# jan-van-bergen/GPU-Raytracer

Hardware: AMD Instinct MI355X
Metric: Mrays/s (primary+secondary) + ms/frame, Sponza 1920x1080 4spp BVH8 (higher is better)
Workload: dtype f32

## Files before the change

gpu-raytracer_amd/__init__.py:

```python
import ctypes
import fcntl
import os
import tarfile
import tempfile
from ctypes import POINTER, byref, c_char_p, c_double, c_float, c_int, c_int32, c_size_t, c_uint8, c_uint32, c_void_p

import numpy as np

_HERE = os.path.dirname(os.path.abspath(__file__))
REPO_ROOT = os.path.dirname(_HERE)
ASSET_DIR = os.path.join(REPO_ROOT, "assets")
DEVICE_LIB_PATH = os.environ.get("GRT_DEVICE_LIB") or os.path.join(_HERE, "csrc", "libgrt_device.so")
HOST_LIB_PATH = os.path.join(_HERE, "host", "libgrt_host.so")

RT_MAX_BOUNCES = 128
RT_BATCH_SIZE = 1080 * 720
AOV_RADIANCE, AOV_RADIANCE_DIRECT, AOV_RADIANCE_INDIRECT, AOV_ALBEDO, AOV_NORMAL, AOV_POSITION, AOV_COUNT = range(7)
MATERIAL_LIGHT, MATERIAL_DIFFUSE, MATERIAL_PLASTIC, MATERIAL_DIELECTRIC, MATERIAL_CONDUCTOR = range(5)
FILTER_BOX, FILTER_TENT, FILTER_GAUSSIAN = range(3)


class GPUConfig(ctypes.Structure):
    _fields_ = [("reconstruction_filter", c_int32), ("aov_mask", c_uint32), ("num_bounces", c_int32),
                ("enable_mipmapping", c_int32), ("enable_next_event_estimation", c_int32),
# ... 23 lines not shown

_device = None
_host = None


def device_lib():
    global _device
    if _device is None:
        if not os.path.exists(DEVICE_LIB_PATH):
            raise DeviceLibraryMissing("%s is missing -- run `python __graft_entry__.py` (build()) first" % DEVICE_LIB_PATH)
        lib = ctypes.CDLL(DEVICE_LIB_PATH, mode=ctypes.RTLD_GLOBAL)
        if hasattr(lib, "rt_abi_version") and lib.rt_abi_version() != 17:
            raise DeviceLibraryMissing("%s has ABI version %d, this front end was written for 17 -- rebuild (python __graft_entry__.py)" % (DEVICE_LIB_PATH, lib.rt_abi_version()))
        lib.rt_last_error.restype = c_char_p
        lib.rt_last_error.argtypes = [c_void_p]
        lib.rt_version.restype = c_char_p
        lib.rt_create.argtypes = [c_int, POINTER(c_void_p)]
        lib.rt_destroy.argtypes = [c_void_p]
        fp, u32p, u8p = POINTER(c_float), POINTER(c_uint32), POINTER(c_uint8)
        lib.rt_trace_rays.argtypes = [c_void_p] + [c_void_p] * 6 + [c_size_t, c_void_p, c_int, POINTER(c_float)]
        lib.rt_trace_shadow_rays.argtypes = [c_void_p] + [c_void_p] * 7 + [c_size_t, c_void_p, c_int, POINTER(c_float)]
        lib.rt_trace_stream_rays.argtypes = [c_void_p, c_int] + [c_void_p] * 6 + [c_size_t, c_void_p] + [c_void_p] * 7 + [c_size_t, c_void_p, c_void_p, c_void_p]
        lib.rt_generate_rays.argtypes = [c_void_p, c_int, c_int, c_int] + [c_void_p] * 7
        lib.rt_random_samples.argtypes = [c_void_p, c_int, c_void_p, c_size_t, c_uint32, c_uint32, c_void_p]
        lib.rt_sample_texture.argtypes = [c_void_p, c_int, c_int, c_void_p, c_size_t, c_void_p]
        lib.rt_sample_table.argtypes = [c_void_p, c_void_p, c_int, c_int, c_int, c_int, c_void_p, c_size_t, c_void_p]
        lib.rt_sample_sky.argtypes = [c_void_p, c_void_p, c_size_t, c_void_p]
        lib.rt_sample_sky_distribution.argtypes = [c_void_p, c_void_p, c_size_t, c_void_p]
        lib.rt_sky_pdf.argtypes = [c_void_p, c_void_p, c_size_t, c_void_p]
        lib.rt_bsdf_eval.argtypes = [c_void_p, c_int, c_void_p, c_size_t, c_void_p]
        lib.rt_bsdf_sample.argtypes = [c_void_p, c_int, c_void_p, c_size_t, c_void_p]
        lib.rt_sample_lights.argtypes = [c_void_p, c_void_p, c_size_t, c_int, c_void_p]
        lib.rt_sort_rays.argtypes = [c_void_p, c_int, c_int, c_int, c_void_p, c_size_t, c_void_p, c_size_t, c_void_p, c_size_t, c_size_t, c_uint32] + [c_void_p] * 9
        lib.rt_upload_lights.argtypes = [c_void_p, c_void_p, c_void_p, c_size_t, c_void_p, c_void_p, c_void_p, c_size_t, c_float]
        lib.rt_upload_material_normal_maps.argtypes = [c_void_p, c_void_p, c_size_t]
        lib.rt_set_bvh_type.argtypes = [c_void_p, c_int]
        lib.rt_upload_material_opacity.argtypes = [c_void_p, c_void_p, c_void_p, c_void_p, c_size_t]
        lib.rt_read_material_opacity.argtypes = [c_void_p, c_int, c_void_p, c_size_t, POINTER(c_int), POINTER(c_int)]
        lib.rt_perturb_normals.argtypes = [c_void_p, c_int, c_void_p, c_size_t, c_void_p]
        lib.rt_set_sky_sampling.argtypes = [c_void_p, c_float]
        lib.rt_set_sky.argtypes = [c_void_p, c_void_p, c_int, c_int, c_float]
        lib.rt_upload_media.argtypes = [c_void_p, c_void_p, c_size_t]
        lib.rt_upload_instances.argtypes = [c_void_p] + [c_void_p] * 5 + [c_size_t]
        lib.rt_upload_materials.argtypes = [c_void_p, c_void_p, c_void_p, c_size_t]
        lib.rt_set_pixel_query.argtypes = [c_void_p, c_int]
        lib.rt_set_svgf_matrices.argtypes = [c_void_p, c_void_p, c_void_p]
# ... 714 lines not shown
    _dev_check(ctx, device_lib().rt_trace_shadow_rays(ctx, o[0].ctypes.data, o[1].ctypes.data, o[2].ctypes.data, d[0].ctypes.data, d[1].ctypes.data, d[2].ctypes.data, m.ctypes.data, n, occluded.ctypes.data, repeat, byref(ms)))
    return occluded, ms.value


def trace_stream_rays(ctx, iteration, origin, direction, hits, shadow_origin, shadow_direction, max_distance, counting=False):
    o, d = _f32(origin).reshape(3, -1), _f32(direction).reshape(3, -1)
    so, sd, m = _f32(shadow_origin).reshape(3, -1), _f32(shadow_direction).reshape(3, -1), _f32(max_distance).reshape(-1)
    n, k = o.shape[1], so.shape[1]
    if d.shape[1] != n or sd.shape[1] != k or m.size != k:
        raise ValueError("trace_stream_rays: ray arrays of different lengths")
    out = np.array(hits, np.uint32, order="C", copy=True).reshape(n, 4)
    light = np.zeros(k, np.float32)
    stats = np.zeros(10, np.uint64) if counting else None
    info = np.zeros(4, np.int32)
    _dev_check(ctx, device_lib().rt_trace_stream_rays(ctx, iteration, o[0].ctypes.data, o[1].ctypes.data, o[2].ctypes.data, d[0].ctypes.data, d[1].ctypes.data, d[2].ctypes.data, n, out.ctypes.data,
                                                      so[0].ctypes.data, so[1].ctypes.data, so[2].ctypes.data, sd[0].ctypes.data, sd[1].ctypes.data, sd[2].ctypes.data, m.ctypes.data, k, light.ctypes.data,
                                                      stats.ctypes.data if counting else None, info.ctypes.data))
    if counting:
        names = ("nodes", "triangles", "instances_transformed", "instances_identity", "rays")
        stats = {kind: {name: int(stats[5 * j + i]) for i, name in enumerate(names)} for j, kind in enumerate(("closest", "shadow"))}
    return out, light, stats, info


def generate_rays(ctx, sample_index, pixel_offset, pixel_count):
    o = np.zeros((3, pixel_count), np.float32)
    d = np.zeros((3, pixel_count), np.float32)
    px = np.zeros(pixel_count, np.uint32)
    _dev_check(ctx, device_lib().rt_generate_rays(ctx, sample_index, pixel_offset, pixel_count, o[0].ctypes.data, o[1].ctypes.data, o[2].ctypes.data, d[0].ctypes.data, d[1].ctypes.data, d[2].ctypes.data, px.ctypes.data))
    return o, d, px


def random_samples(ctx, dimension, pixel_indices, bounce, sample_index):
    px = np.ascontiguousarray(pixel_indices, dtype=np.uint32)
    out = np.zeros((px.size, 2), np.float32)
    _dev_check(ctx, device_lib().rt_random_samples(ctx, dimension, px.ctypes.data, px.size, bounce, sample_index, out.ctypes.data))
    return out


def sample_texture(ctx, texture_index, filter, args):
    a = _f32(args).reshape(-1, 8)
    out = np.zeros((a.shape[0], 4), np.float32)
    _dev_check(ctx, device_lib().rt_sample_texture(ctx, texture_index, filter, a.ctypes.data, a.shape[0], out.ctypes.data))
    return out


def sample_table(ctx, table, coords):
# ... 282 lines not shown
```

gpu-raytracer_amd/csrc/kernels_shade.hip:

```cpp
#include "rt_shading.h"

#ifndef RT_SHADE_BLOCK
#define RT_SHADE_BLOCK 256
#endif
#ifndef RT_SHADE_WAVES
#define RT_SHADE_WAVES 4
#endif
#ifndef RT_SHADE_ONE_APPEND
#define RT_SHADE_ONE_APPEND 1
#endif
#ifndef RT_OCTANT_BUCKETS
#define RT_OCTANT_BUCKETS 1
#endif
#if RT_OCTANT_BUCKETS
#define RT_RAY_BUCKET(d) direction_octant(d)
#else
#define RT_RAY_BUCKET(d) 0u
#endif
#ifndef RT_SORT_BLOCK
#define RT_SORT_BLOCK 1024
#endif
#ifndef RT_SORT_WAVES
#define RT_SORT_WAVES 8
#endif
// ... 46 lines not shown
	origin = mk3(p.camera.position[0], p.camera.position[1], p.camera.position[2]) + offset;
}

__global__ void __launch_bounds__(RT_SHADE_BLOCK) kernel_generate(RtParams p, int sample_index, int pixel_offset, int pixel_count) {
	const int ray_count = pixel_count * p.batch_samples;
	if (blockIdx.x == 0 && threadIdx.x == 0) p.sizes->trace[0] = ray_count;
	for (int index = blockIdx.x * blockDim.x + threadIdx.x; index < ray_count; index += gridDim.x * blockDim.x) {
		int sample_in_batch = index / pixel_count;
		int index_offset = rt_map_pixel(p, index - sample_in_batch * pixel_count + pixel_offset);
		int x = index_offset % p.screen_width;
		int y = index_offset / p.screen_width;
		int pixel_index = x + y * p.screen_pitch;
		unsigned virtual_pixel = unsigned(sample_in_batch) * p.frame_pixels + unsigned(pixel_index);

		f3 origin, direction;
		camera_generate_ray(p, int(virtual_pixel), sample_index, x, y, origin, direction, sample_index + sample_in_batch);

		store3(p.trace[0].origin,    index, origin);
		store3(p.trace[0].direction, index, direction);
		p.trace[0].pixel_index_and_flags[index] = virtual_pixel;
	}
}

__global__ void __launch_bounds__(RT_SHADE_BLOCK) kernel_generate_stream(RtParams p, int sample_index, int pixel_offset, int pixel_count, int slot_base, int queue_offset, int block_width, int band_rows) {
	const int ray_count = pixel_count * p.batch_samples;
	const RtTraceBuffer & out = p.trace[p.stream_iteration & 1];
	const int base = p.stream->trace_count[p.stream_iteration & 1] + queue_offset;
	for (int index = blockIdx.x * blockDim.x + threadIdx.x; index < ray_count; index += gridDim.x * blockDim.x) {
		int sample_in_batch = index / pixel_count;
		int index_offset = rt_map_pixel(p, index - sample_in_batch * pixel_count + pixel_offset);
		int x = index_offset % p.screen_width;
		int y = index_offset / p.screen_width;
		if (band_rows > 0) {
			int band = y / band_rows;
			int rows = min(band_rows, p.screen_height - band * band_rows);
			int in_band = index_offset - band * band_rows * p.screen_width;
			if (band_rows == 8 && block_width == 8 && rows == 8 && (in_band >> 6) * 8 + 8 <= p.screen_width) {
				x = (in_band >> 6) * 8 + (in_band & 7);
				y = band * 8 + ((in_band >> 3) & 7);
			} else {
				int block = in_band / (block_width * rows);
				int in_block = in_band - block * block_width * rows;
				int columns = min(block_width, p.screen_width - block * block_width);
				x = block * block_width + in_block % columns;
				y = band * band_rows + in_block / columns;
			}
		}
		int pixel_index = x + y * p.screen_pitch;
		unsigned slot = unsigned(slot_base + sample_in_batch);
		unsigned virtual_pixel = slot * p.frame_pixels + unsigned(pixel_index);

		f3 origin, direction;
		camera_generate_ray(p, int(virtual_pixel), sample_index + sample_in_batch - int(slot), x, y, origin, direction, sample_index + sample_in_batch);

		store3(out.origin,    base + index, origin);
		store3(out.direction, base + index, direction);
		out.pixel_index_and_flags[base + index] = virtual_pixel;
	}
}

__global__ void __launch_bounds__(256) kernel_stream_advance(RtStreamControl * control, int iteration, int generated, volatile int * progress, int reset_ring_first, int reset_ring_count) {
	for (int k = int(threadIdx.x); k < reset_ring_count * RT_STAT_KINDS * RT_MAX_BOUNCES; k += int(blockDim.x))
		(&control->stats[(reset_ring_first + k / (RT_STAT_KINDS * RT_MAX_BOUNCES)) % RT_STREAM_SUBMISSIONS][0][0])[k % (RT_STAT_KINDS * RT_MAX_BOUNCES)] = 0;
	const int q = iteration & 1;
	for (int k = int(threadIdx.x); k < 2 * RT_ENDGAME_MAX_WAVES; k += int(blockDim.x)) (&control->endgame[q][0][0])[k] = 0;
	if (threadIdx.x != 0) return;
	int total = control->trace_count[q] + generated;
	control->trace_count[q] = total;
	control->trace_count[q ^ 1] = 0;
	for (int m = 0; m < 4; m++) control->material_count[m] = 0;
	control->shadow_count[q] = 0;
	control->cursor[q][0] = 0; control->cursor[q][1] = 0;
	if (progress) { progress[1] = total; __threadfence_system(); progress[0] = iteration; }
}

__global__ void kernel_expand_bc1(const uint2 * __restrict__ blocks, uchar4 * __restrict__ texels, size_t texel_count) {
// ... 1184 lines not shown
		case 2: hipLaunchKernelGGL(sky ? kernel_material_dielectric_sky_nmap : kernel_material_dielectric_nmap, grid, block, 0, stream, p, bounce, sample_index); break;
		case 3: hipLaunchKernelGGL(sky ? kernel_material_conductor_sky_nmap  : kernel_material_conductor_nmap,  grid, block, 0, stream, p, bounce, sample_index); break;
	}
}
void rt_launch_material(const RtParams & p, int material_slot, int bounce, int sample_index, hipStream_t stream) {
	dim3 grid(2048), block(RT_SHADE_BLOCK);
	if (p.normal_map_slots & (1 << material_slot)) { launch_material_nmap(p, material_slot, bounce, sample_index, stream); return; }
	if (p.sky_nee_share > 0.0f) {
		switch (material_slot) {
			case 0: hipLaunchKernelGGL(p.textures_compressed ? kernel_material_diffuse_sky : kernel_material_diffuse_texels_sky, grid, block, 0, stream, p, bounce, sample_index); break;
			case 1: hipLaunchKernelGGL(p.textures_compressed ? kernel_material_plastic_sky : kernel_material_plastic_texels_sky, grid, block, 0, stream, p, bounce, sample_index); break;
			case 2: hipLaunchKernelGGL(kernel_material_dielectric_sky, grid, block, 0, stream, p, bounce, sample_index); break;
			case 3: hipLaunchKernelGGL(kernel_material_conductor_sky,  grid, block, 0, stream, p, bounce, sample_index); break;
		}
		return;
	}
	switch (material_slot) {
		case 0: if (p.textures_compressed) hipLaunchKernelGGL(kernel_material_diffuse, grid, block, 0, stream, p, bounce, sample_index); else hipLaunchKernelGGL(kernel_material_diffuse_texels, grid, block, 0, stream, p, bounce, sample_index); break;
		case 1: if (p.textures_compressed) hipLaunchKernelGGL(kernel_material_plastic, grid, block, 0, stream, p, bounce, sample_index); else hipLaunchKernelGGL(kernel_material_plastic_texels, grid, block, 0, stream, p, bounce, sample_index); break;
		case 2: hipLaunchKernelGGL(kernel_material_dielectric, grid, block, 0, stream, p, bounce, sample_index); break;
		case 3: hipLaunchKernelGGL(kernel_material_conductor,  grid, block, 0, stream, p, bounce, sample_index); break;
	}
}
void rt_launch_generate_stream(const RtParams & p, int sample_index, int pixel_offset, int pixel_count, int slot_base, int queue_offset, int block_width, int band_rows, hipStream_t stream) {
	hipLaunchKernelGGL(kernel_generate_stream, dim3(streaming_grid(pixel_count * p.batch_samples)), dim3(RT_SHADE_BLOCK), 0, stream, p, sample_index, pixel_offset, pixel_count, slot_base, queue_offset, block_width, band_rows);
}
void rt_launch_stream_advance(RtStreamControl * control, int iteration, int generated, int * progress, int reset_ring_first, int reset_ring_count, hipStream_t stream) {
	hipLaunchKernelGGL(kernel_stream_advance, dim3(1), dim3(256), 0, stream, control, iteration, generated, (volatile int *)progress, reset_ring_first, reset_ring_count);
}
#ifndef RT_STREAM_SHADE_GRID
#define RT_STREAM_SHADE_GRID 8192
#endif
#ifndef RT_STREAM_SORT_GRID
#define RT_STREAM_SORT_GRID 2048
#endif
void rt_launch_sort_stream(const RtParams & p, hipStream_t stream) {
	hipLaunchKernelGGL(p.sky_nee_share > 0.0f ? kernel_sort_stream_sky : kernel_sort_stream, dim3(RT_STREAM_SORT_GRID * RT_SHADE_BLOCK / RT_SORT_BLOCK), dim3(RT_SORT_BLOCK), 0, stream, p);
}
static void launch_material_stream_nmap(const RtParams & p, int material_slot, hipStream_t stream) {
	dim3 grid(RT_STREAM_SHADE_GRID), block(RT_SHADE_BLOCK);
	const bool sky = p.sky_nee_share > 0.0f, compressed = p.textures_compressed != 0;
	switch (material_slot) {
		case 0: hipLaunchKernelGGL(sky ? (compressed ? kernel_material_diffuse_stream_sky_nmap : kernel_material_diffuse_stream_texels_sky_nmap) : (compressed ? kernel_material_diffuse_stream_nmap : kernel_material_diffuse_stream_texels_nmap), grid, block, 0, stream, p); break;
		case 1: hipLaunchKernelGGL(sky ? (compressed ? kernel_material_plastic_stream_sky_nmap : kernel_material_plastic_stream_texels_sky_nmap) : (compressed ? kernel_material_plastic_stream_nmap : kernel_material_plastic_stream_texels_nmap), grid, block, 0, stream, p); break;
		case 2: hipLaunchKernelGGL(sky ? kernel_material_dielectric_stream_sky_nmap : kernel_material_dielectric_stream_nmap, grid, block, 0, stream, p); break;
		case 3: hipLaunchKernelGGL(sky ? kernel_material_conductor_stream_sky_nmap  : kernel_material_conductor_stream_nmap,  grid, block, 0, stream, p); break;
	}
}
// ... 57 lines not shown
```

gpu-raytracer_amd/csrc/rt_api.hip:

```cpp
#include "rt_tlas_build.h"
#include <dlfcn.h>
#include "rt_types.h"
#include "rt_tlas_build.h"

#include <algorithm>
#include <cmath>
#include <cstdarg>
#include <cstdio>
#include <cstdlib>
#include <cstring>
#include <deque>
#include <memory>
#include <string>
#include <vector>

static thread_local std::string g_global_error;

static void warn_if_streams_share_queues(int streams_needed) {
	static bool warned = false;
	if (warned) return;
	const char * value = getenv("GPU_MAX_HW_QUEUES");
	const int queues = value ? atoi(value) : 4;
	if (queues >= streams_needed) return;
	warned = true;
// ... 40 lines not shown
	int * ray_cursors = nullptr;
	void * spill[2] = { nullptr, nullptr };
	int * counter_totals = nullptr;
	RtBufferSizes * pinned_counters = nullptr;
	void * aov_framebuffer[RT_AOV_COUNT] = { };
	int aov_samples = 1;
	void * gbuffers[3] = { };
	hipEvent_t ev_gbuffers = nullptr;
};

#define RT_SCENE_VERSIONS 12
struct SceneRing {
	void * device[RT_SCENE_VERSIONS] = { };
	void * pinned[RT_SCENE_VERSIONS] = { };
	hipEvent_t copied[RT_SCENE_VERSIONS] = { };
	size_t capacity = 0;
	size_t bytes = 0;
	int current = -1;
	unsigned users[RT_SCENE_VERSIONS] = { };
	hipEvent_t last_use[RT_SCENE_VERSIONS][RT_MAX_SAMPLE_SLOTS] = { };
};

#define RT_STREAM_BATCH_PATHS     (1920 * 1080 * 4)
#define RT_STREAM_MAX_BATCH       8
#define RT_STREAM_PROGRESS_RING   64
#define RT_STREAM_RUN_AHEAD       4
#define RT_STREAM_TABLE_SNAPSHOTS 8
#define RT_STREAM_HISTORY_ROWS    4096
#define RT_STREAM_STATS_ROW       (RT_STAT_KINDS * RT_MAX_BOUNCES)

struct StreamSubmission {
	int first_sample, sample_count, slot_base, ring, birth, last, paths;
	int range_offset, range_count, tile_pixels, tile_first, tile_stride;
};

struct PathStream {
	bool created = false;
	hipStream_t stream = nullptr;
	hipEvent_t ev_idle = nullptr;
	WavefrontQueues queues;
	RtStreamControl * control = nullptr;
	RtStreamTable * table_device = nullptr;
	RtStreamTable table_host;
	RtStreamTable * table_staging = nullptr; hipEvent_t table_copied[RT_STREAM_TABLE_SNAPSHOTS] = { }; int table_next = 0;
	void * spill = nullptr;
	void * aov_framebuffer[RT_AOV_COUNT] = { }; int frame_slots = 0;
	void * gbuffers[3] = { };
// ... 1918 lines not shown
		for (int j = 0; j < sub.sample_count; j++) s.slot_used[sub.slot_base + j] = false;
		s.last_completed_ring = sub.ring;
		s.submissions_completed++;
	}
	RT_HIP(ctx, hipEventRecord(s.ev_idle, st));
	return RT_OK;
}

static int stream_sync_tlas(rt_context * ctx) {
	if (ctx->tlas_version_in_nodes == ctx->tlas_version) return RT_OK;
	if (!ctx->params.tlas_nodes || ctx->params.tlas_node_count <= 0) {
		ctx->tlas_version_in_nodes = ctx->tlas_version; return RT_OK;
	}
	if (!ctx->bvh8_nodes || size_t(ctx->params.tlas_node_count) > ctx->bvh8_node_count) return fail(ctx, RT_ERROR_NOT_READY, "rt_render_samples: the TLAS does not fit the node slots the geometry reserves for it");
	if (ctx->tlas_node_bytes != 80) return fail(ctx, RT_ERROR_INVALID_ARG, "rt_render_samples: the merged wavefront needs the TLAS as 80-byte CWBVH nodes (rt_upload_tlas); select RT_SCHEDULER_SLOTS for other BVH types");
	if (ctx->params.tlas_node_count > ctx->lowest_blas_root) return fail(ctx, RT_ERROR_INVALID_ARG, "rt_render_samples: a BLAS root (node %d) lies inside the %d node slots the merged wavefront copies the TLAS into; reserve them in front of the BLAS nodes or select RT_SCHEDULER_SLOTS", ctx->lowest_blas_root, ctx->params.tlas_node_count);
	hipStream_t st = ctx->path_stream.stream;
	RT_HIP(ctx, hipStreamWaitEvent(st, ctx->ev_scene, 0));
	RT_HIP(ctx, hipMemcpyAsync(ctx->bvh8_nodes, ctx->params.tlas_nodes, size_t(ctx->params.tlas_node_count) * 80, hipMemcpyDeviceToDevice, st));
	ctx->tlas_version_in_nodes = ctx->tlas_version;
	return RT_OK;
}

static int stream_generate(rt_context * ctx, const StreamSubmission & sub) {
	PathStream & s = ctx->path_stream;
	hipStream_t st = s.stream;
	RT_HIP(ctx, hipStreamWaitEvent(st, ctx->ev_scene, 0));
	RtParams pg = stream_params(ctx, s.iteration);
	pg.batch_samples = sub.sample_count;
	pg.tile_pixels = sub.tile_pixels; pg.tile_first = sub.tile_first; pg.tile_stride = sub.tile_stride;
	RT_HIP(ctx, hipEventRecord(s.ev_begin[sub.ring], st));
	stage_mark(ctx, STAGE_GENERATE, st);
	span_mark(ctx, SPAN_GENERATE, st);
	const int order = 8;
	const int frame = pg.screen_width * pg.screen_height;
	const bool whole_bands = sub.tile_pixels > 0 ? sub.tile_pixels % (order * pg.screen_width) == 0 : (sub.range_offset == 0 && sub.range_count == frame);
	rt_launch_generate_stream(pg, sub.first_sample, sub.range_offset, sub.range_count, sub.slot_base, int(s.pending_paths), whole_bands ? order : 0, whole_bands ? order : 0, st);
	span_mark(ctx, SPAN_GENERATE, st);
	s.pending++; s.pending_paths += sub.paths;
	return RT_OK;
}

static int stream_enqueue_iteration(rt_context * ctx) {
	PathStream & s = ctx->path_stream;
	const int i = s.iteration;
	hipStream_t st = s.stream;
	if (i - RT_STREAM_RUN_AHEAD >= 0) RT_HIP(ctx, hipEventSynchronize(s.iteration_done[(i - RT_STREAM_RUN_AHEAD) % RT_STREAM_PROGRESS_RING]));
	RtParams p = stream_params(ctx, i);
	const int generated = int(s.pending_paths);
	s.pending = 0; s.pending_paths = 0;
	if (s.table_dirty) {
		int snapshot = s.table_next; s.table_next = (s.table_next + 1) % RT_STREAM_TABLE_SNAPSHOTS;
		RT_HIP(ctx, hipEventSynchronize(s.table_copied[snapshot]));
		s.table_staging[snapshot] = s.table_host;
		RT_HIP(ctx, hipMemcpyAsync(s.table_device, &s.table_staging[snapshot], sizeof(RtStreamTable), hipMemcpyHostToDevice, st));
		RT_HIP(ctx, hipEventRecord(s.table_copied[snapshot], st));
		s.table_dirty = false;
	}
	rt_launch_stream_advance(s.control, i, generated, s.progress + 2 * (i % RT_STREAM_PROGRESS_RING), s.reset_ring_first, s.reset_ring_count, st);
	s.reset_ring_count = 0;
	s.generated[i % RT_STREAM_PROGRESS_RING] = generated;
	RT_HIP(ctx, hipEventRecord(s.iteration_done[i % RT_STREAM_PROGRESS_RING], st));
	stage_mark(ctx, STAGE_TRACE, st);
	span_mark(ctx, SPAN_TRACE, st);
	rt_launch_trace_stream(p, ctx->trace_statistics ? ctx->trace_stats : nullptr, st);
	span_mark(ctx, SPAN_TRACE, st);
	if (ctx->trace_statistics && ctx->stream_history_rows < RT_STREAM_HISTORY_ROWS)
		RT_HIP(ctx, hipMemcpyAsync(ctx->stream_history + size_t(10) * ctx->stream_history_rows++, ctx->trace_stats, 10 * sizeof(unsigned long long), hipMemcpyDeviceToHost, st));
	stage_mark(ctx, STAGE_SORT, st);
	span_mark(ctx, SPAN_SORT, st);
	rt_launch_sort_stream(p, st);
	span_mark(ctx, SPAN_SORT, st);
// ... 71 lines not shown
		s.slot_used[slot_base + k] = true;
		s.table_host.slots[slot_base + k] = { sample_index + k, sub.birth, sub.ring, k };
	}
	s.next_slot = (slot_base + sample_count) % s.frame_slots;
	s.table_host.submission_birth[sub.ring] = sub.birth;
	if (s.reset_ring_count == 0) s.reset_ring_first = sub.ring;
	s.reset_ring_count++; s.table_dirty = true;
	if (ctx->trace_statistics && s.in_flight.empty()) {
		RT_HIP(ctx, hipMemsetAsync(ctx->trace_stats, 0, 10 * sizeof(unsigned long long), s.stream));
		ctx->stream_history_rows = 0;
	}
	s.in_flight.push_back(sub);
	if (ctx->params.config.enable_svgf && s.gbuffers[0]) {
		const void * from[3];
		for (int i = 0; i < 3; i++) {
			if (s.last_gbuffer_slot >= 0) from[i] = (char *)s.gbuffers[i] + ctx->frame_pixels * gbuffer_pixel_bytes[i] * size_t(s.last_gbuffer_slot);
			else from[i] = (ctx->last_slot > 0 && ctx->slots[ctx->last_slot].gbuffers[i]) ? ctx->slots[ctx->last_slot].gbuffers[i] : ctx->svgf_buffers[i];
			void * to = (char *)s.gbuffers[i] + ctx->frame_pixels * gbuffer_pixel_bytes[i] * size_t(slot_base);
			if (from[i] && from[i] != to) RT_HIP(ctx, hipMemcpyAsync(to, from[i], ctx->frame_pixels * gbuffer_pixel_bytes[i], hipMemcpyDeviceToDevice, s.stream));
		}
		s.last_gbuffer_slot = slot_base;
	}
	status = stream_sync_tlas(ctx); if (status) return status;
	status = stream_generate(ctx, sub); if (status) return status;
	if (s.pending < batch && s.pending_paths < batch_paths) return RT_OK;
	return stream_enqueue_iteration(ctx);
}

static int finish_slot_submission(rt_context * ctx, int slot_index) {
	SampleSlot & slot = ctx->slots[slot_index];
	hipStream_t st = slot.stream;
	RT_HIP(ctx, hipMemcpyAsync(slot.pinned_counters, slot.counter_totals, 6 * RT_MAX_BOUNCES * sizeof(int), hipMemcpyDeviceToHost, st));
	RT_HIP(ctx, hipEventRecord(slot.ev_frame_end, st));
	RT_HIP(ctx, hipEventRecord(slot.ev_done, st));
	int status = mark_scene_versions_in_use(ctx, slot_index, st); if (status) return status;
	ctx->last_slot = slot_index;
	RT_HIP(ctx, hipGetLastError());
	return RT_OK;
}

extern "C" {

int rt_render_sample(rt_context * ctx, int sample_index) { return rt_render_samples(ctx, sample_index, 1); }

int rt_render_samples(rt_context * ctx, int sample_index, int sample_count) {
	RT_REQUIRE(ctx, ctx, "rt_render_sample: NULL context");
	RT_REQUIRE(ctx, sample_count >= 1 && sample_count <= RT_MAX_BATCH_SAMPLES, "rt_render_samples: sample_count must be 1..16");
// ... 418 lines not shown
	    !shadow.origin.x || !shadow.origin.y || !shadow.origin.z || !shadow.direction.x || !shadow.direction.y || !shadow.direction.z ||
	    !shadow.max_distance || !shadow.illumination_and_pixel_index || !radiance || !control || (stats10 && !stats))
		return fail(ctx, RT_ERROR_HIP, "rt_trace_stream_rays: device allocation failed");
	if (shadow_count) RT_HIP(ctx, hipMemset(radiance, 0, shadow_count * 16));
	if (stats) RT_HIP(ctx, hipMemset(stats, 0, 10 * sizeof(unsigned long long)));

	RtParams p = stream_params(ctx, iteration);
	p.trace[q] = trace;
	p.shadow = shadow;
	p.stream = control;
	for (int a = 0; a < RT_AOV_COUNT; a++) p.aovs[a].framebuffer = nullptr;
	p.aovs[RT_AOV_RADIANCE].framebuffer = radiance;
	rt_trace_stream_launch_info(p, stats != nullptr, info);
	rt_launch_trace_stream(p, stats, ps.stream);
	RT_HIP(ctx, hipGetLastError());
	RT_HIP(ctx, hipStreamSynchronize(ps.stream));
	if (closest_count) RT_HIP(ctx, hipMemcpy(hits, trace.hits, closest_count * 16, hipMemcpyDeviceToHost));
	if (shadow_count) {
		std::vector<float4> added(shadow_count);
		RT_HIP(ctx, hipMemcpy(added.data(), radiance, shadow_count * 16, hipMemcpyDeviceToHost));
		for (size_t i = 0; i < shadow_count; i++) shadow_light[i] = added[i].x;
	}
	if (stats10) RT_HIP(ctx, hipMemcpy(stats10, stats, 10 * sizeof(unsigned long long), hipMemcpyDeviceToHost));
	return RT_OK;
}

int rt_generate_rays(rt_context * ctx, int sample_index, int pixel_offset, int pixel_count,
                     float * ox, float * oy, float * oz, float * dx, float * dy, float * dz, uint32_t * pixel_index_and_flags) {
	RT_REQUIRE(ctx, ctx && ox && oy && oz && dx && dy && dz && pixel_index_and_flags, "rt_generate_rays: NULL argument");
	RT_REQUIRE(ctx, pixel_count >= 0, "rt_generate_rays: negative pixel_count");
	(void)hipSetDevice(ctx->device);
	if (!ctx->params.pmj_samples || ctx->frame_pixels == 0) return fail(ctx, RT_ERROR_NOT_READY, "rt_generate_rays: RNG tables not uploaded or rt_resize not called");
	RT_HIP(ctx, quiesce(ctx));
	int s = ensure_queues(ctx); if (s) return s;
	if (size_t(pixel_count) > ctx->slots[0].queues.capacity) return fail(ctx, RT_ERROR_OUT_OF_RANGE, "rt_generate_rays: pixel_count %d exceeds the queue capacity %zu", pixel_count, ctx->slots[0].queues.capacity);
	rt_launch_generate(ctx->params, sample_index, pixel_offset, pixel_count, ctx->stream);
	RT_HIP(ctx, hipGetLastError());
	RT_HIP(ctx, quiesce(ctx));
	const RtTraceBuffer & t = ctx->params.trace[0];
	size_t bytes = size_t(pixel_count) * 4;
	RT_HIP(ctx, hipMemcpy(ox, t.origin.x, bytes, hipMemcpyDeviceToHost));
	RT_HIP(ctx, hipMemcpy(oy, t.origin.y, bytes, hipMemcpyDeviceToHost));
	RT_HIP(ctx, hipMemcpy(oz, t.origin.z, bytes, hipMemcpyDeviceToHost));
	RT_HIP(ctx, hipMemcpy(dx, t.direction.x, bytes, hipMemcpyDeviceToHost));
	RT_HIP(ctx, hipMemcpy(dy, t.direction.y, bytes, hipMemcpyDeviceToHost));
	RT_HIP(ctx, hipMemcpy(dz, t.direction.z, bytes, hipMemcpyDeviceToHost));
// ... 399 lines not shown
```

gpu-raytracer_amd/csrc/rt_types.h:

```cpp
#pragma once
#include <hip/hip_runtime.h>
#include <stdint.h>

#include "../../include/gpu_raytracer_amd.h"

#define RT_WAVE_SIZE 64
#define RT_INFINITY __builtin_huge_valf()

struct RtVec3SoA { float * x, * y, * z; };

struct RtTraceBuffer {
	RtVec3SoA origin, direction;
	uint4   * hits;
	float   * cone_angle, * cone_width;
	int     * medium;
	unsigned * pixel_index_and_flags;
	RtVec3SoA throughput;
	float   * last_pdf;
};

struct RtMaterialBuffer {
	RtVec3SoA direction;
	uint4   * hits;
	float   * cone_angle, * cone_width;
// ... 149 lines not shown
}

struct RtPathInfo { int bounce, submission; unsigned sample_index_for_rng; bool first_of_submission; };
__device__ __forceinline__ RtPathInfo rt_stream_path_info(const RtParams & p, unsigned virtual_pixel) {
	unsigned slot;
	rt_split_virtual_pixel(p, virtual_pixel, slot);
	RtStreamSlot e = p.stream_table->slots[slot];
	RtPathInfo info;
	info.bounce = p.stream_iteration - e.birth_iteration;
	info.submission = e.submission;
	info.sample_index_for_rng = unsigned(e.sample_index) - slot;
	info.first_of_submission = e.index_in_submission == 0;
	return info;
}

#define RT_FLAG_ALLOW_NEE     (1u << 31)
#define RT_FLAG_INSIDE_MEDIUM (1u << 30)
#define RT_FLAGS_ALL          (RT_FLAG_ALLOW_NEE | RT_FLAG_INSIDE_MEDIUM)
#define RT_SHADOW_FLAG_BOUNCE_0 (1u << 30)

void rt_launch_generate(const RtParams & p, int sample_index, int pixel_offset, int pixel_count, hipStream_t stream);
void rt_launch_expand_bc1(const uint2 * blocks, uchar4 * texels, size_t block_count, hipStream_t stream);
void rt_launch_trace(const RtParams & p, int bounce, hipStream_t stream);
void rt_launch_generate_stream(const RtParams & p, int sample_index, int pixel_offset, int pixel_count, int slot_base, int queue_offset, int block_width, int band_rows, hipStream_t stream);
void rt_launch_stream_advance(RtStreamControl * control, int iteration, int generated, int * progress, int reset_ring_first, int reset_ring_count, hipStream_t stream);
void rt_launch_trace_stream(const RtParams & p, unsigned long long * stats, hipStream_t stream);
enum { RT_STREAM_KERNEL_GENERAL = 0, RT_STREAM_KERNEL_FLAT = 1, RT_STREAM_KERNEL_FLAT_SKIP = 2, RT_STREAM_KERNEL_COUNTING = 3,
       RT_STREAM_KERNEL_GENERAL_MASK = 4, RT_STREAM_KERNEL_FLAT_MASK = 5, RT_STREAM_KERNEL_FLAT_SKIP_MASK = 6, RT_STREAM_KERNEL_COUNTING_MASK = 7 };
void rt_trace_stream_launch_info(const RtParams & p, bool stats, int32_t * info);
void rt_launch_sort_stream(const RtParams & p, hipStream_t stream);
void rt_launch_material_stream(const RtParams & p, int material_slot, hipStream_t stream);
void rt_launch_trace_shadow(const RtParams & p, int bounce, hipStream_t stream);
void rt_launch_ambient_occlusion(const RtParams & p, int sample_index, float ao_radius, hipStream_t stream);
void rt_launch_trace_shadow_ao(const RtParams & p, hipStream_t stream);
void rt_launch_sort(const RtParams & p, int bounce, int sample_index, hipStream_t stream);
void rt_launch_material(const RtParams & p, int material_slot, int bounce, int sample_index, hipStream_t stream);
void rt_launch_accumulate(const RtParams & p, float frames_accumulated, int pixel_offset, int pixel_count, hipStream_t stream);
#define RT_SVGF_YOUNG_HEADER 16
#define RT_ACCUMULATE_GROUP 8
struct RtAccumulateGroup { int count; int first_sample[RT_ACCUMULATE_GROUP], sample_count[RT_ACCUMULATE_GROUP], slot_base[RT_ACCUMULATE_GROUP]; };
void rt_launch_accumulate_group(const RtParams & p, const RtAccumulateGroup & group, int pixel_offset, int pixel_count, hipStream_t stream);
void rt_launch_svgf_taa(const RtParams & p, int sample_index, hipStream_t stream, void (*mark)(void * user, int svgf_kernel, hipStream_t stream) = nullptr, void * user = nullptr);
void rt_launch_random(const RtParams & p, int dimension, const unsigned * pixel_indices, int count, unsigned bounce, unsigned sample_index, float2 * out, hipStream_t stream);
void rt_launch_sample_texture(const RtParams & p, int texture_index, int filter, const float * args, int count, float4 * out, hipStream_t stream);
void rt_launch_sample_table(const float * table, int nx, int ny, int nz, int dims, const float * coords, int count, float * out, hipStream_t stream);
void rt_launch_sample_sky(const RtParams & p, const float * directions, int count, float * out, hipStream_t stream);
#define RT_BSDF_PROBE_IN  24
// ... 19 lines not shown
```

include/gpu_raytracer_amd.h:

```cpp
#ifndef GPU_RAYTRACER_AMD_H
#define GPU_RAYTRACER_AMD_H

#include <stddef.h>
#include <stdint.h>

#ifdef __cplusplus
extern "C" {
#endif

#define RT_MAX_BOUNCES                  128
#define RT_BATCH_SIZE                   (1080 * 720)
#define RT_PMJ_NUM_SEQUENCES            64
#define RT_PMJ_NUM_SAMPLES_PER_SEQUENCE 4096
#define RT_BLUE_NOISE_NUM_TEXTURES      16
#define RT_BLUE_NOISE_TEXTURE_DIM       128
#define RT_MAX_ATROUS_ITERATIONS        10
#define RT_LUT_DIELECTRIC_DIM           16
#define RT_LUT_CONDUCTOR_DIM            32
#define RT_INVALID                      (-1)

typedef enum rt_status {
	RT_OK                 =  0,
	RT_ERROR_INVALID_ARG  = -1,
	RT_ERROR_NO_DEVICE    = -2,
// ... 211 lines not shown
                     float * ox, float * oy, float * oz, float * dx, float * dy, float * dz,
                     uint32_t * pixel_index_and_flags);
int rt_random_samples(rt_context * ctx, int dimension, const uint32_t * pixel_indices, size_t count,
                      uint32_t bounce, uint32_t sample_index, float * out_xy);
int rt_sample_texture(rt_context * ctx, int texture_index, int filter, const float * args, size_t count, float * out_rgba);
int rt_sample_table(rt_context * ctx, const float * table, int nx, int ny, int nz, int dims, const float * coords, size_t count, float * out);
int rt_sample_sky(rt_context * ctx, const float * directions, size_t count, float * out_rgb);
int rt_sample_sky_distribution(rt_context * ctx, const float * uv, size_t count, float * out_xyz_pdf);
int rt_sky_pdf(rt_context * ctx, const float * directions, size_t count, float * out_pdf);
int rt_bsdf_eval(rt_context * ctx, int material_type, const float * probes, size_t count, float * out);
int rt_bsdf_sample(rt_context * ctx, int material_type, const float * probes, size_t count, float * out);
#define RT_LIGHT_SAMPLE_OUT 16
int rt_sample_lights(rt_context * ctx, const float * probes, size_t count, int use_lds, float * out);
#define RT_NORMAL_PROBE_IN 48
int rt_perturb_normals(rt_context * ctx, int texture_index, const float * probes, size_t count, float * out);
#define RT_SORT_TRACE_WORDS    20
#define RT_SORT_MATERIAL_WORDS 16
int rt_sort_rays(rt_context * ctx, int merged, int step, int sample_index, const uint32_t * trace_in, size_t count,
                 const int32_t * slot_table, size_t slot_count, const int32_t * submission_birth,
                 size_t capacity, size_t frame_slots, uint32_t sentinel,
                 uint32_t * trace_out, uint32_t * material_out, int32_t * counters6,
                 float * aov_frames, float * gbuffer_normal_and_depth, int32_t * gbuffer_mesh_id_and_triangle_id, float * gbuffer_screen_position_prev,
                 int32_t * pixel_query2, int32_t * stats);
int rt_measure_stream_bandwidth(rt_context * ctx, size_t bytes, int repeat, float * out_gbps);

#ifdef __cplusplus
}
#endif
#endif
```

Baseline: 3912.

## Defer and merge stream ray generation into grouped launches with pixel-run interleaving

Ray generation for submitted frames is deferred until the iteration is enqueued. Consecutive submissions that share a pixel range are merged into a single generate launch. Within a launch, samples are interleaved in runs of 64 pixels, so neighbouring queue entries hold the same pixels across samples rather than one whole frame per sample. This is meant to improve ray coherence for traversal and to cut launch overhead, at the cost of extra index arithmetic. It also adds an API to read back the generated order and an optional supertile remap, which is off by default.

```diff
diff --git a/gpu-raytracer_amd/__init__.py b/gpu-raytracer_amd/__init__.py
--- a/gpu-raytracer_amd/__init__.py
+++ b/gpu-raytracer_amd/__init__.py
@@ -69,6 +69,7 @@
         lib.rt_trace_shadow_rays.argtypes = [c_void_p] + [c_void_p] * 7 + [c_size_t, c_void_p, c_int, POINTER(c_float)]
         lib.rt_trace_stream_rays.argtypes = [c_void_p, c_int] + [c_void_p] * 6 + [c_size_t, c_void_p] + [c_void_p] * 7 + [c_size_t, c_void_p, c_void_p, c_void_p]
         lib.rt_generate_rays.argtypes = [c_void_p, c_int, c_int, c_int] + [c_void_p] * 7
+        lib.rt_generate_stream_order.argtypes = [c_void_p, c_void_p, c_size_t, c_size_t, POINTER(c_size_t)] + [c_void_p] * 7
         lib.rt_random_samples.argtypes = [c_void_p, c_int, c_void_p, c_size_t, c_uint32, c_uint32, c_void_p]
         lib.rt_sample_texture.argtypes = [c_void_p, c_int, c_int, c_void_p, c_size_t, c_void_p]
         lib.rt_sample_table.argtypes = [c_void_p, c_void_p, c_int, c_int, c_int, c_int, c_void_p, c_size_t, c_void_p]
@@ -829,6 +830,18 @@
     return out, light, stats, info
 
 
+def generate_stream_order(ctx, submissions, pixel_count):
+    subs = np.ascontiguousarray(np.array(submissions, np.int32).reshape(-1, 2))
+    capacity = int(pixel_count) * int(subs[:, 1].clip(0).sum())
+    o = np.zeros((3, max(capacity, 1)), np.float32)
+    d = np.zeros((3, max(capacity, 1)), np.float32)
+    px = np.zeros(max(capacity, 1), np.uint32)
+    entries = c_size_t(0)
+    _dev_check(ctx, device_lib().rt_generate_stream_order(ctx, subs.ctypes.data if len(subs) else None, len(subs), capacity, byref(entries), px.ctypes.data,
+                                                          o[0].ctypes.data, o[1].ctypes.data, o[2].ctypes.data, d[0].ctypes.data, d[1].ctypes.data, d[2].ctypes.data))
+    return px[:entries.value], o[:, :entries.value], d[:, :entries.value]
+
+
 def generate_rays(ctx, sample_index, pixel_offset, pixel_count):
     o = np.zeros((3, pixel_count), np.float32)
     d = np.zeros((3, pixel_count), np.float32)
diff --git a/gpu-raytracer_amd/csrc/kernels_shade.hip b/gpu-raytracer_amd/csrc/kernels_shade.hip
--- a/gpu-raytracer_amd/csrc/kernels_shade.hip
+++ b/gpu-raytracer_amd/csrc/kernels_shade.hip
@@ -92,13 +92,49 @@
 	}
 }
 
-__global__ void __launch_bounds__(RT_SHADE_BLOCK) kernel_generate_stream(RtParams p, int sample_index, int pixel_offset, int pixel_count, int slot_base, int queue_offset, int block_width, int band_rows) {
-	const int ray_count = pixel_count * p.batch_samples;
+#ifndef RT_PRIMARY_RUN
+#define RT_PRIMARY_RUN 64
+#endif
+#ifndef RT_PRIMARY_SUPERTILE
+#define RT_PRIMARY_SUPERTILE 0
+#endif
+__global__ void __launch_bounds__(RT_SHADE_BLOCK) kernel_generate_stream(RtParams p, RtGenerateGroup group, int pixel_offset, int pixel_count, int queue_offset, int block_width, int band_rows) {
+	const int samples = group.samples;
+	const int ray_count = pixel_count * samples;
+	const int tail = pixel_count % RT_PRIMARY_RUN;
+	const int whole = (pixel_count - tail) * samples;
 	const RtTraceBuffer & out = p.trace[p.stream_iteration & 1];
 	const int base = p.stream->trace_count[p.stream_iteration & 1] + queue_offset;
 	for (int index = blockIdx.x * blockDim.x + threadIdx.x; index < ray_count; index += gridDim.x * blockDim.x) {
-		int sample_in_batch = index / pixel_count;
-		int index_offset = rt_map_pixel(p, index - sample_in_batch * pixel_count + pixel_offset);
+		int sample_in_group, pixel;
+		if (index < whole) {
+			int chunk = index / (RT_PRIMARY_RUN * samples);
+			int in_chunk = index - chunk * (RT_PRIMARY_RUN * samples);
+			sample_in_group = in_chunk / RT_PRIMARY_RUN;
+			pixel = chunk * RT_PRIMARY_RUN + in_chunk % RT_PRIMARY_RUN;
+		} else {
+			sample_in_group = (index - whole) / tail;
+			pixel = pixel_count - tail + (index - whole) % tail;
+		}
+		int sample_index = 0, slot_index = 0, rest = sample_in_group;
+		#pragma unroll
+		for (int k = 0; k < RT_STREAM_MAX_BATCH; k++) {
+			if (rest >= 0 && rest < group.sample_count[k]) { sample_index = group.first_sample[k] + rest; slot_index = group.slot_base[k] + rest; }
+			rest -= group.sample_count[k];
+		}
+#if RT_PRIMARY_SUPERTILE
+		if (band_rows == 8 && block_width == 8 && p.tile_pixels == 0 && pixel_offset == 0 && pixel_count == p.screen_width * p.screen_height && p.screen_width % (8 * RT_PRIMARY_SUPERTILE) == 0 && p.screen_height % 8 == 0) {
+			const int across = p.screen_width / 8, bands = p.screen_height / 8;
+			int patch = pixel >> 6;
+			int tile_row = patch / (across * RT_PRIMARY_SUPERTILE);
+			int in_row = patch - tile_row * across * RT_PRIMARY_SUPERTILE;
+			int rows_here = min(RT_PRIMARY_SUPERTILE, bands - tile_row * RT_PRIMARY_SUPERTILE);
+			int tile = in_row / (RT_PRIMARY_SUPERTILE * rows_here), in_tile = in_row - tile * RT_PRIMARY_SUPERTILE * rows_here;
+			int band_of_patch = tile_row * RT_PRIMARY_SUPERTILE + in_tile / RT_PRIMARY_SUPERTILE, column = tile * RT_PRIMARY_SUPERTILE + in_tile % RT_PRIMARY_SUPERTILE;
+			pixel = (band_of_patch * across + column) * 64 + (pixel & 63);
+		}
+#endif
+		int index_offset = rt_map_pixel(p, pixel + pixel_offset);
 		int x = index_offset % p.screen_width;
 		int y = index_offset / p.screen_width;
 		if (band_rows > 0) {
@@ -117,11 +153,11 @@
 			}
 		}
 		int pixel_index = x + y * p.screen_pitch;
-		unsigned slot = unsigned(slot_base + sample_in_batch);
+		unsigned slot = unsigned(slot_index);
 		unsigned virtual_pixel = slot * p.frame_pixels + unsigned(pixel_index);
 
 		f3 origin, direction;
-		camera_generate_ray(p, int(virtual_pixel), sample_index + sample_in_batch - int(slot), x, y, origin, direction, sample_index + sample_in_batch);
+		camera_generate_ray(p, int(virtual_pixel), sample_index - int(slot), x, y, origin, direction, sample_index);
 
 		store3(out.origin,    base + index, origin);
 		store3(out.direction, base + index, direction);
@@ -1352,8 +1388,8 @@
 		case 3: hipLaunchKernelGGL(kernel_material_conductor,  grid, block, 0, stream, p, bounce, sample_index); break;
 	}
 }
-void rt_launch_generate_stream(const RtParams & p, int sample_index, int pixel_offset, int pixel_count, int slot_base, int queue_offset, int block_width, int band_rows, hipStream_t stream) {
-	hipLaunchKernelGGL(kernel_generate_stream, dim3(streaming_grid(pixel_count * p.batch_samples)), dim3(RT_SHADE_BLOCK), 0, stream, p, sample_index, pixel_offset, pixel_count, slot_base, queue_offset, block_width, band_rows);
+void rt_launch_generate_stream(const RtParams & p, const RtGenerateGroup & group, int pixel_offset, int pixel_count, int queue_offset, int block_width, int band_rows, hipStream_t stream) {
+	hipLaunchKernelGGL(kernel_generate_stream, dim3(streaming_grid(pixel_count * group.samples)), dim3(RT_SHADE_BLOCK), 0, stream, p, group, pixel_offset, pixel_count, queue_offset, block_width, band_rows);
 }
 void rt_launch_stream_advance(RtStreamControl * control, int iteration, int generated, int * progress, int reset_ring_first, int reset_ring_count, hipStream_t stream) {
 	hipLaunchKernelGGL(kernel_stream_advance, dim3(1), dim3(256), 0, stream, control, iteration, generated, (volatile int *)progress, reset_ring_first, reset_ring_count);
diff --git a/gpu-raytracer_amd/csrc/rt_api.hip b/gpu-raytracer_amd/csrc/rt_api.hip
--- a/gpu-raytracer_amd/csrc/rt_api.hip
+++ b/gpu-raytracer_amd/csrc/rt_api.hip
@@ -86,7 +86,6 @@
 };
 
 #define RT_STREAM_BATCH_PATHS     (1920 * 1080 * 4)
-#define RT_STREAM_MAX_BATCH       8
 #define RT_STREAM_PROGRESS_RING   64
 #define RT_STREAM_RUN_AHEAD       4
 #define RT_STREAM_TABLE_SNAPSHOTS 8
@@ -2051,22 +2050,59 @@
 	return RT_OK;
 }
 
-static int stream_generate(rt_context * ctx, const StreamSubmission & sub) {
+struct GenerateLaunch {
+	RtGenerateGroup group;
+	int range_offset, range_count, tile_pixels, tile_first, tile_stride;
+	int queue_offset;
+	int first, count;
+};
+static int stream_group_generation(const StreamSubmission * subs, int count, std::vector<GenerateLaunch> & launches) {
+	long long offset = 0;
+	for (int first = 0; first < count; ) {
+		const StreamSubmission & head = subs[first];
+		GenerateLaunch g = { };
+		g.range_offset = head.range_offset; g.range_count = head.range_count; g.tile_pixels = head.tile_pixels; g.tile_first = head.tile_first; g.tile_stride = head.tile_stride;
+		g.queue_offset = int(offset); g.first = first;
+		int k = first;
+		for (; k < count && g.group.count < RT_STREAM_MAX_BATCH; k++) {
+			const StreamSubmission & sub = subs[k];
+			if (sub.range_offset != head.range_offset || sub.range_count != head.range_count || sub.tile_pixels != head.tile_pixels || sub.tile_first != head.tile_first || sub.tile_stride != head.tile_stride) break;
+			g.group.first_sample[g.group.count] = sub.first_sample; g.group.slot_base[g.group.count] = sub.slot_base; g.group.sample_count[g.group.count] = sub.sample_count;
+			g.group.count++; g.group.samples += sub.sample_count;
+		}
+		g.count = k - first;
+		offset += (long long)g.range_count * g.group.samples;
+		launches.push_back(g);
+		first = k;
+	}
+	return int(offset);
+}
+static void stream_launch_generation(const RtParams & p, const GenerateLaunch & g, hipStream_t st) {
+	RtParams pg = p;
+	pg.tile_pixels = g.tile_pixels; pg.tile_first = g.tile_first; pg.tile_stride = g.tile_stride;
+	const int order = 8;
+	const int frame = pg.screen_width * pg.screen_height;
+	const bool whole_bands = g.tile_pixels > 0 ? g.tile_pixels % (order * pg.screen_width) == 0 : (g.range_offset == 0 && g.range_count == frame);
+	rt_launch_generate_stream(pg, g.group, g.range_offset, g.range_count, g.queue_offset, whole_bands ? order : 0, whole_bands ? order : 0, st);
+}
+
+static int stream_generate_pending(rt_context * ctx, const RtParams & p) {
 	PathStream & s = ctx->path_stream;
+	if (s.pending == 0) return RT_OK;
 	hipStream_t st = s.stream;
 	RT_HIP(ctx, hipStreamWaitEvent(st, ctx->ev_scene, 0));
-	RtParams pg = stream_params(ctx, s.iteration);
-	pg.batch_samples = sub.sample_count;
-	pg.tile_pixels = sub.tile_pixels; pg.tile_first = sub.tile_first; pg.tile_stride = sub.tile_stride;
-	RT_HIP(ctx, hipEventRecord(s.ev_begin[sub.ring], st));
-	stage_mark(ctx, STAGE_GENERATE, st);
-	span_mark(ctx, SPAN_GENERATE, st);
-	const int order = 8;
-	const int frame = pg.screen_width * pg.screen_height;
-	const bool whole_bands = sub.tile_pixels > 0 ? sub.tile_pixels % (order * pg.screen_width) == 0 : (sub.range_offset == 0 && sub.range_count == frame);
-	rt_launch_generate_stream(pg, sub.first_sample, sub.range_offset, sub.range_count, sub.slot_base, int(s.pending_paths), whole_bands ? order : 0, whole_bands ? order : 0, st);
-	span_mark(ctx, SPAN_GENERATE, st);
-	s.pending++; s.pending_paths += sub.paths;
+	StreamSubmission subs[RT_STREAM_MAX_BATCH];
+	const int count = s.pending;
+	for (int k = 0; k < count; k++) subs[k] = s.in_flight[s.in_flight.size() - size_t(count) + size_t(k)];
+	std::vector<GenerateLaunch> launches;
+	stream_group_generation(subs, count, launches);
+	for (const GenerateLaunch & g : launches) {
+		for (int k = 0; k < g.count; k++) RT_HIP(ctx, hipEventRecord(s.ev_begin[subs[g.first + k].ring], st));
+		stage_mark(ctx, STAGE_GENERATE, st);
+		span_mark(ctx, SPAN_GENERATE, st);
+		stream_launch_generation(p, g, st);
+		span_mark(ctx, SPAN_GENERATE, st);
+	}
 	return RT_OK;
 }
 
@@ -2077,6 +2113,7 @@
 	if (i - RT_STREAM_RUN_AHEAD >= 0) RT_HIP(ctx, hipEventSynchronize(s.iteration_done[(i - RT_STREAM_RUN_AHEAD) % RT_STREAM_PROGRESS_RING]));
 	RtParams p = stream_params(ctx, i);
 	const int generated = int(s.pending_paths);
+	{ int status = stream_generate_pending(ctx, p); if (status) return status; }
 	s.pending = 0; s.pending_paths = 0;
 	if (s.table_dirty) {
 		int snapshot = s.table_next; s.table_next = (s.table_next + 1) % RT_STREAM_TABLE_SNAPSHOTS;
@@ -2194,7 +2231,7 @@
 		s.last_gbuffer_slot = slot_base;
 	}
 	status = stream_sync_tlas(ctx); if (status) return status;
-	status = stream_generate(ctx, sub); if (status) return status;
+	s.pending++; s.pending_paths += sub.paths;
 	if (s.pending < batch && s.pending_paths < batch_paths) return RT_OK;
 	return stream_enqueue_iteration(ctx);
 }
@@ -2659,6 +2696,65 @@
 		for (size_t i = 0; i < shadow_count; i++) shadow_light[i] = added[i].x;
 	}
 	if (stats10) RT_HIP(ctx, hipMemcpy(stats10, stats, 10 * sizeof(unsigned long long), hipMemcpyDeviceToHost));
+	return RT_OK;
+}
+
+int rt_generate_stream_order(rt_context * ctx, const int32_t * submissions, size_t submission_count, size_t capacity, size_t * entries,
+                             uint32_t * pixel_index_and_flags, float * ox, float * oy, float * oz, float * dx, float * dy, float * dz) {
+	RT_REQUIRE(ctx, ctx != nullptr, "rt_generate_stream_order: NULL context");
+	RT_REQUIRE(ctx, submissions && submission_count >= 1, "rt_generate_stream_order: empty submission list");
+	RT_REQUIRE(ctx, submission_count <= size_t(RT_STREAM_SUBMISSIONS), "rt_generate_stream_order: more than 128 submissions");
+	RT_REQUIRE(ctx, entries && pixel_index_and_flags && ox && oy && oz && dx && dy && dz, "rt_generate_stream_order: NULL output array");
+	(void)hipSetDevice(ctx->device);
+	int s = check_ready(ctx, "rt_generate_stream_order", NEED_RNG | NEED_FRAME); if (s) return s;
+	int range_offset = 0, range_count = 0;
+	s = resolve_pixel_range(ctx, "rt_generate_stream_order", &range_offset, &range_count); if (s) return s;
+	const size_t slot_limit = std::min<size_t>(RT_STREAM_SAMPLE_SLOTS, ((size_t(1) << 30) - 1) / ctx->frame_pixels);
+	std::vector<StreamSubmission> subs(submission_count);
+	size_t samples = 0;
+	for (size_t k = 0; k < submission_count; k++) {
+		const int first_sample = submissions[2 * k], sample_count = submissions[2 * k + 1];
+		RT_REQUIRE(ctx, first_sample >= 0 && sample_count >= 1 && sample_count <= RT_MAX_BATCH_SAMPLES, "rt_generate_stream_order: a submission needs first_sample >= 0 and 1..16 samples");
+		StreamSubmission sub = { };
+		sub.first_sample = first_sample; sub.sample_count = sample_count; sub.slot_base = int(samples);
+		sub.range_offset = range_offset; sub.range_count = range_count; sub.paths = range_count * sample_count;
+		sub.tile_pixels = ctx->params.tile_pixels; sub.tile_first = ctx->params.tile_first; sub.tile_stride = ctx->params.tile_stride;
+		subs[k] = sub;
+		samples += size_t(sample_count);
+	}
+	if (samples > slot_limit) return fail(ctx, RT_ERROR_OUT_OF_RANGE, "rt_generate_stream_order: %zu samples of a %zu pixel frame exceed the %zu sample slots of the merged wavefront", samples, ctx->frame_pixels, slot_limit);
+	const size_t total = size_t(range_count) * samples;
+	if (total > capacity || total >= (size_t(1) << 30)) return fail(ctx, RT_ERROR_OUT_OF_RANGE, "rt_generate_stream_order: %zu queue entries exceed the capacity %zu of the output arrays (or 2^30)", total, capacity);
+	RT_HIP(ctx, quiesce(ctx));
+	s = stream_create(ctx); if (s) return s;
+	PathStream & ps = ctx->path_stream;
+	*entries = total;
+	if (total == 0) return RT_OK;
+
+	TempBuffers tmp(ctx);
+	RtTraceBuffer trace = { };
+	trace.origin    = { (float *)tmp.get(total * 4, nullptr), (float *)tmp.get(total * 4, nullptr), (float *)tmp.get(total * 4, nullptr) };
+	trace.direction = { (float *)tmp.get(total * 4, nullptr), (float *)tmp.get(total * 4, nullptr), (float *)tmp.get(total * 4, nullptr) };
+	trace.pixel_index_and_flags = (unsigned *)tmp.get(total * 4, nullptr);
+	std::unique_ptr<RtStreamControl> control_host(new RtStreamControl());
+	RtStreamControl * control = (RtStreamControl *)tmp.get(sizeof(RtStreamControl), control_host.get());
+	if (!trace.origin.x || !trace.origin.y || !trace.origin.z || !trace.direction.x || !trace.direction.y || !trace.direction.z || !trace.pixel_index_and_flags || !control)
+		return fail(ctx, RT_ERROR_HIP, "rt_generate_stream_order: device allocation failed");
+	RtParams p = stream_params(ctx, 0);
+	p.trace[0] = trace;
+	p.stream = control;
+	std::vector<GenerateLaunch> launches;
+	stream_group_generation(subs.data(), int(submission_count), launches);
+	for (const GenerateLaunch & g : launches) stream_launch_generation(p, g, ps.stream);
+	RT_HIP(ctx, hipGetLastError());
+	RT_HIP(ctx, hipStreamSynchronize(ps.stream));
+	RT_HIP(ctx, hipMemcpy(ox, trace.origin.x, total * 4, hipMemcpyDeviceToHost));
+	RT_HIP(ctx, hipMemcpy(oy, trace.origin.y, total * 4, hipMemcpyDeviceToHost));
+	RT_HIP(ctx, hipMemcpy(oz, trace.origin.z, total * 4, hipMemcpyDeviceToHost));
+	RT_HIP(ctx, hipMemcpy(dx, trace.direction.x, total * 4, hipMemcpyDeviceToHost));
+	RT_HIP(ctx, hipMemcpy(dy, trace.direction.y, total * 4, hipMemcpyDeviceToHost));
+	RT_HIP(ctx, hipMemcpy(dz, trace.direction.z, total * 4, hipMemcpyDeviceToHost));
+	RT_HIP(ctx, hipMemcpy(pixel_index_and_flags, trace.pixel_index_and_flags, total * 4, hipMemcpyDeviceToHost));
 	return RT_OK;
 }
 
diff --git a/gpu-raytracer_amd/csrc/rt_types.h b/gpu-raytracer_amd/csrc/rt_types.h
--- a/gpu-raytracer_amd/csrc/rt_types.h
+++ b/gpu-raytracer_amd/csrc/rt_types.h
@@ -195,7 +195,9 @@
 void rt_launch_generate(const RtParams & p, int sample_index, int pixel_offset, int pixel_count, hipStream_t stream);
 void rt_launch_expand_bc1(const uint2 * blocks, uchar4 * texels, size_t block_count, hipStream_t stream);
 void rt_launch_trace(const RtParams & p, int bounce, hipStream_t stream);
-void rt_launch_generate_stream(const RtParams & p, int sample_index, int pixel_offset, int pixel_count, int slot_base, int queue_offset, int block_width, int band_rows, hipStream_t stream);
+#define RT_STREAM_MAX_BATCH 8
+struct RtGenerateGroup { int count, samples; int first_sample[RT_STREAM_MAX_BATCH], slot_base[RT_STREAM_MAX_BATCH], sample_count[RT_STREAM_MAX_BATCH]; };
+void rt_launch_generate_stream(const RtParams & p, const RtGenerateGroup & group, int pixel_offset, int pixel_count, int queue_offset, int block_width, int band_rows, hipStream_t stream);
 void rt_launch_stream_advance(RtStreamControl * control, int iteration, int generated, int * progress, int reset_ring_first, int reset_ring_count, hipStream_t stream);
 void rt_launch_trace_stream(const RtParams & p, unsigned long long * stats, hipStream_t stream);
 enum { RT_STREAM_KERNEL_GENERAL = 0, RT_STREAM_KERNEL_FLAT = 1, RT_STREAM_KERNEL_FLAT_SKIP = 2, RT_STREAM_KERNEL_COUNTING = 3,
diff --git a/include/gpu_raytracer_amd.h b/include/gpu_raytracer_amd.h
--- a/include/gpu_raytracer_amd.h
+++ b/include/gpu_raytracer_amd.h
@@ -257,6 +257,8 @@
                  uint32_t * trace_out, uint32_t * material_out, int32_t * counters6,
                  float * aov_frames, float * gbuffer_normal_and_depth, int32_t * gbuffer_mesh_id_and_triangle_id, float * gbuffer_screen_position_prev,
                  int32_t * pixel_query2, int32_t * stats);
+int rt_generate_stream_order(rt_context * ctx, const int32_t * submissions, size_t submission_count, size_t capacity, size_t * entries,
+                             uint32_t * pixel_index_and_flags, float * ox, float * oy, float * oz, float * dx, float * dy, float * dz);
 int rt_measure_stream_bandwidth(rt_context * ctx, size_t bytes, int repeat, float * out_gbps);
 
 #ifdef __cplusplus
```

Result: no change. 3912 (-0.0%).
